# takahiroharada/OCLRadixSort

Measured on AMD Instinct MI355X. Metric: Gkeys/s on uniform-random u32 keys; achieved % of HBM-read roofline, higher is better.
Workload: dtype u32; 1 GPU; Key-only RadixSort32, 67108864 uniform-random u32 keys (splitmix64 hi32, seed 123+step), 1xMI355X, in place; keys_per_gpu=67108864, parallelism=1 GPU, sort_algo=auto, digit_bits=8

## Files before the change

oclradixsort_amd/csrc/finish16_kernels.hpp:

```cpp
#pragma once
#include <hip/hip_runtime.h>
#include <stdint.h>

#include "hybrid_kernels.hpp"

namespace adlhip {

template <int R2>
struct Finish16Cfg {
    static constexpr int CAP = 128 * R2;
    static constexpr size_t PER_WAVE = 2 * CAP + 256 * 4;
};

__device__ __forceinline__ uint32_t finish16_index(uint32_t p) { return (p & ~127u) | ((p & 63u) << 1) | ((p >> 6) & 1u); }

__device__ __forceinline__ void finish16_lds_order() { __builtin_amdgcn_fence(__ATOMIC_ACQ_REL, "wavefront"); }

template <int RR>
__device__ __forceinline__ void finish16_rows(const uint32_t* __restrict__ src32, uint32_t* __restrict__ out, uint32_t m, int lane,
                                              uint16_t* __restrict__ buf16, uint32_t* __restrict__ cnt, uint32_t low_bits, uint32_t hi)
{
    constexpr int L = RR - 1;
    const bool a_lo = 2u * (uint32_t)(64 * L + lane) < m, a_hi = 2u * (uint32_t)(64 * L + lane) + 1u < m;
    const bool b_lo = (uint32_t)(128 * L + lane) < m, b_hi = (uint32_t)(128 * L + 64 + lane) < m;
    uint32_t kp[RR];
#pragma unroll
    for (int j = 0; j < RR; ++j)
        if (j < L || a_lo) kp[j] = __builtin_nontemporal_load(src32 + j * 64 + lane);
    bool placed = false;
    const int npass = ((int)low_bits + 7) / 8;
    int sb = 0;
    const uint32_t* buf32 = reinterpret_cast<const uint32_t*>(buf16);
    for (int p = 0; p < npass; ++p) {
        const int nb = ((int)low_bits - sb + (npass - p - 1)) / (npass - p);
        const uint32_t mask = (1u << nb) - 1u;
        const bool v_lo = placed ? b_lo : a_lo, v_hi = placed ? b_hi : a_hi;
        auto dlo = [&](uint32_t x) -> uint32_t { return (x >> sb) & mask; };
        auto dhi = [&](uint32_t x) -> uint32_t { return (x >> (16 + sb)) & mask; };
        {
            const uint32_t d0 = (uint32_t)__builtin_amdgcn_readfirstlane((int)dlo(kp[0]));
            bool same = true;
#pragma unroll
            for (int j = 0; j < RR; ++j) {
                if (j < L || v_lo) same &= dlo(kp[j]) == d0;
                if (j < L || v_hi) same &= dhi(kp[j]) == d0;
            }
            if (__all(same)) {
                sb += nb;
                continue;
            }
        }
        const u32x4 z = {0u, 0u, 0u, 0u};
        *reinterpret_cast<u32x4*>(cnt + 4 * lane) = z;
        uint32_t rk[RR];
#pragma unroll
        for (int j = 0; j < RR; ++j) {
            uint32_t r0 = 0u, r1 = 0u;
            if (j < L || v_lo) r0 = __hip_atomic_fetch_add(&cnt[dlo(kp[j])], 1u, __ATOMIC_RELAXED, __HIP_MEMORY_SCOPE_WAVEFRONT);
            if (j < L || v_hi) r1 = __hip_atomic_fetch_add(&cnt[dhi(kp[j])], 1u, __ATOMIC_RELAXED, __HIP_MEMORY_SCOPE_WAVEFRONT);
            rk[j] = r0 | (r1 << 16);
        }
        {
            const u32x4 c = *reinterpret_cast<const u32x4*>(cnt + 4 * lane);
            const uint32_t s4 = c.x + c.y + c.z + c.w;
            const uint32_t ex = wave_incl_scan_u32(s4) - s4;
            u32x4 o;
            o.x = ex;
            o.y = ex + c.x;
            o.z = o.y + c.y;
            o.w = o.z + c.z;
            *reinterpret_cast<u32x4*>(cnt + 4 * lane) = o;
        }
        finish16_lds_order();
#pragma unroll
        for (int j = 0; j < RR; ++j) {
            uint32_t p0 = 0u, p1 = 0u;
            if (j < L || v_lo) p0 = cnt[dlo(kp[j])] + (rk[j] & 0xffffu);
            if (j < L || v_hi) p1 = cnt[dhi(kp[j])] + (rk[j] >> 16);
            if (j < L || v_lo) buf16[finish16_index(p0)] = (uint16_t)kp[j];
            if (j < L || v_hi) buf16[finish16_index(p1)] = (uint16_t)(kp[j] >> 16);
        }
        finish16_lds_order();
#pragma unroll
        for (int j = 0; j < RR; ++j)
            if (j < L || b_lo) kp[j] = buf32[j * 64 + lane];
        placed = true;
        sb += nb;
    }
    if (placed) {
#pragma unroll
        for (int j = 0; j < RR; ++j) {
            if (j < L || b_lo) __builtin_nontemporal_store(hi | (kp[j] & 0xffffu), out + 128 * j + lane);
            if (j < L || b_hi) __builtin_nontemporal_store(hi | (kp[j] >> 16), out + 128 * j + 64 + lane);
        }
    } else {
#pragma unroll
        for (int j = 0; j < RR; ++j) {
            if (j < L || a_lo) out[2 * (64 * j + lane)] = hi | (kp[j] & 0xffffu);
            if (j < L || a_hi) out[2 * (64 * j + lane) + 1] = hi | (kp[j] >> 16);
        }
    }
}

template <int RR, int R2>
__device__ __forceinline__ void finish16_dispatch(int rows2, const uint32_t* __restrict__ src32, uint32_t* __restrict__ out, uint32_t m,
                                                  int lane, uint16_t* __restrict__ buf16, uint32_t* __restrict__ cnt, uint32_t low_bits,
                                                  uint32_t hi)
{
    if constexpr (RR >= R2) {
        finish16_rows<R2>(src32, out, m, lane, buf16, cnt, low_bits, hi);
    } else {
        if (rows2 <= RR) finish16_rows<RR>(src32, out, m, lane, buf16, cnt, low_bits, hi);
        else finish16_dispatch<RR + 1, R2>(rows2, src32, out, m, lane, buf16, cnt, low_bits, hi);
    }
}

template <int R2, int WAVES>
__global__ __launch_bounds__(64 * WAVES) void wave_finish16_kernel(const uint16_t* __restrict__ slab, uint32_t* __restrict__ out,
                                                                    const uint32_t* __restrict__ seg_off,
                                                                    const uint32_t* __restrict__ seg_cnt, uint32_t stride,
                                                                    const uint32_t* __restrict__ gate, const uint32_t* __restrict__ dyn,
                                                                    uint32_t num_segments, uint32_t* fault)
{
    if (gate && *gate != 0u) return;
    using C = Finish16Cfg<R2>;
    extern __shared__ __attribute__((aligned(16))) unsigned char smem[];
    const int lane = (int)threadIdx.x & 63;
    const int w = (int)threadIdx.x >> 6;
    unsigned char* mine = smem + (size_t)w * C::PER_WAVE;
    uint16_t* __restrict__ buf16 = reinterpret_cast<uint16_t*>(mine);
    uint32_t* __restrict__ cnt = reinterpret_cast<uint32_t*>(mine + 2 * C::CAP);
    const uint32_t seg = (uint32_t)__builtin_amdgcn_readfirstlane((int)(blockIdx.x * (uint32_t)WAVES + (uint32_t)w));
    if (seg >= num_segments) return;
    const uint32_t low_bits = (uint32_t)__builtin_amdgcn_readfirstlane((int)dyn[0]);
    const uint32_t m = (uint32_t)__builtin_amdgcn_readfirstlane((int)seg_cnt[seg]);
    const uint32_t begin = (uint32_t)__builtin_amdgcn_readfirstlane((int)seg_off[seg]);
    if (m == 0u) return;
    if (m > (uint32_t)C::CAP || low_bits > 16u) {
        if (lane == 0) atomicOr(fault + 1, 0x40000u);
        return;
    }
    const uint32_t hi = ((dyn[1] << 16) | seg) << low_bits;
    const uint32_t* src32 = reinterpret_cast<const uint32_t*>(slab + (size_t)seg * stride);
    finish16_dispatch<1, R2>((int)((m + 127u) >> 7), src32, out + begin, m, lane, buf16, cnt, low_bits, hi);
}

}
```

Before: 215.3 Gkeys/s.

## Add single-pass 512-bin finish16 with odd-even transposition cleanup of low bits

When more than 8 low bits remain, the wave-level finisher now counting-sorts the segment on the top 9 bits in one pass instead of two 8-bit passes. Any leftover lower bits are fixed by a bounded number of odd-even transposition rounds in registers, using DPP to exchange across lanes, and it falls back to the multi-pass path when a bin is too large. The LDS tile is padded to avoid bank conflicts and the counter array is enlarged. This removes one full histogram/scan/scatter pass per segment, at the cost of more LDS per wave and the extra sort rounds.

```diff
diff --git a/oclradixsort_amd/csrc/finish16_kernels.hpp b/oclradixsort_amd/csrc/finish16_kernels.hpp
--- a/oclradixsort_amd/csrc/finish16_kernels.hpp
+++ b/oclradixsort_amd/csrc/finish16_kernels.hpp
@@ -6,15 +6,163 @@
 
 namespace adlhip {
 
+constexpr int kFinish16BinBits = 9;
+constexpr int kFinish16MaxRounds = 24;
+
 template <int R2>
 struct Finish16Cfg {
     static constexpr int CAP = 128 * R2;
-    static constexpr size_t PER_WAVE = 2 * CAP + 256 * 4;
+    static constexpr int BINS = 1 << kFinish16BinBits;
+    static constexpr size_t TILE = 256 * (R2 | 1);
+    static constexpr size_t PER_WAVE = TILE + 4 * BINS;
 };
 
 __device__ __forceinline__ uint32_t finish16_index(uint32_t p) { return (p & ~127u) | ((p & 63u) << 1) | ((p >> 6) & 1u); }
 
 __device__ __forceinline__ void finish16_lds_order() { __builtin_amdgcn_fence(__ATOMIC_ACQ_REL, "wavefront"); }
+
+template <int RR>
+__device__ __forceinline__ uint32_t finish16_block_byte(uint32_t p)
+{
+    constexpr uint32_t J = 2 * RR;
+    if constexpr ((RR & 1) != 0) {
+        return 2u * p;
+    } else if constexpr ((J & (J - 1)) == 0) {
+        return 2u * p + 4u * (p / J);
+    } else {
+        constexpr uint32_t MAGIC = (65536u + J - 1u) / J;
+        static_assert(64u * J * (MAGIC * J - 65536u) < 65536u, "the reciprocal is not exact over the tile");
+        return 2u * p + 4u * (__umul24(p, MAGIC) >> 16);
+    }
+}
+
+__device__ __forceinline__ uint32_t finish16_wave_max(uint32_t v)
+{
+    v = max(v, dpp_mov0<0x111, 0xf, 0xf>(v));
+    v = max(v, dpp_mov0<0x112, 0xf, 0xf>(v));
+    v = max(v, dpp_mov0<0x114, 0xf, 0xf>(v));
+    v = max(v, dpp_mov0<0x118, 0xf, 0xf>(v));
+    v = max(v, dpp_mov0<0x142, 0xa, 0xf>(v));
+    v = max(v, dpp_mov0<0x143, 0xc, 0xf>(v));
+    return (uint32_t)__builtin_amdgcn_readlane((int)v, 63);
+}
+
+template <int RR>
+__device__ __forceinline__ bool finish16_bins(const uint32_t (&kp)[RR], uint32_t* __restrict__ out, uint32_t m, int lane,
+                                              uint16_t* __restrict__ buf16, uint32_t* __restrict__ cnt, uint32_t low_bits, uint32_t hi,
+                                              bool a_lo, bool a_hi, bool b_lo, bool b_hi)
+{
+    constexpr int L = RR - 1, J = 2 * RR, S = RR | 1;
+    constexpr int NB = 1 << kFinish16BinBits, PL = NB / 64;
+    static_assert(PL % 4 == 0, "a lane scans its counters as u32x4");
+    const uint32_t bb = low_bits < (uint32_t)kFinish16BinBits ? low_bits : (uint32_t)kFinish16BinBits;
+    const uint32_t sh = low_bits - bb;
+    auto dlo = [&](uint32_t x) -> uint32_t { return (x >> sh) & (uint32_t)(NB - 1); };
+    auto dhi = [&](uint32_t x) -> uint32_t { return (x >> (16u + sh)) & (uint32_t)(NB - 1); };
+    {
+        const uint32_t d0 = (uint32_t)__builtin_amdgcn_readfirstlane((int)dlo(kp[0]));
+        bool same = true;
+#pragma unroll
+        for (int j = 0; j < RR; ++j) {
+            if (j < L || a_lo) same &= dlo(kp[j]) == d0;
+            if (j < L || a_hi) same &= dhi(kp[j]) == d0;
+        }
+        if (__all(same)) return false;
+    }
+    const u32x4 z = {0u, 0u, 0u, 0u};
+#pragma unroll
+    for (int q = 0; q < PL / 4; ++q) *reinterpret_cast<u32x4*>(cnt + PL * lane + 4 * q) = z;
+    uint32_t rk[RR];
+#pragma unroll
+    for (int j = 0; j < RR; ++j) {
+        uint32_t r0 = 0u, r1 = 0u;
+        if (j < L || a_lo) r0 = __hip_atomic_fetch_add(&cnt[dlo(kp[j])], 1u, __ATOMIC_RELAXED, __HIP_MEMORY_SCOPE_WAVEFRONT);
+        if (j < L || a_hi) r1 = __hip_atomic_fetch_add(&cnt[dhi(kp[j])], 1u, __ATOMIC_RELAXED, __HIP_MEMORY_SCOPE_WAVEFRONT);
+        rk[j] = r0 | (r1 << 16);
+    }
+    const bool tail = low_bits > bb;
+    uint32_t rounds;
+    {
+        u32x4 c[PL / 4];
+        uint32_t sum = 0u, big = 0u;
+#pragma unroll
+        for (int q = 0; q < PL / 4; ++q) {
+            c[q] = *reinterpret_cast<const u32x4*>(cnt + PL * lane + 4 * q);
+            sum += c[q].x + c[q].y + c[q].z + c[q].w;
+            big = max(max(big, max(c[q].x, c[q].y)), max(c[q].z, c[q].w));
+        }
+        rounds = finish16_wave_max(big);
+        if (tail && rounds > (uint32_t)kFinish16MaxRounds) return false;
+        uint32_t run = wave_incl_scan_u32(sum) - sum;
+#pragma unroll
+        for (int q = 0; q < PL / 4; ++q) {
+            u32x4 o;
+            o.x = run;
+            o.y = o.x + c[q].x;
+            o.z = o.y + c[q].y;
+            o.w = o.z + c[q].z;
+            run = o.w + c[q].w;
+            *reinterpret_cast<u32x4*>(cnt + PL * lane + 4 * q) = o;
+        }
+    }
+    unsigned char* tile = reinterpret_cast<unsigned char*>(buf16);
+    const bool sort = tail && rounds > 1u;
+    if (sort) {
+        const uint32_t p0 = m + (uint32_t)lane, p1 = p0 + 64u;
+        if (p0 < (uint32_t)(64 * J)) *reinterpret_cast<uint16_t*>(tile + finish16_block_byte<RR>(p0)) = (uint16_t)0xffffu;
+        if (p1 < (uint32_t)(64 * J)) *reinterpret_cast<uint16_t*>(tile + finish16_block_byte<RR>(p1)) = (uint16_t)0xffffu;
+    }
+    finish16_lds_order();
+#pragma unroll
+    for (int j = 0; j < RR; ++j) {
+        uint32_t p0 = 0u, p1 = 0u;
+        if (j < L || a_lo) p0 = cnt[dlo(kp[j])] + (rk[j] & 0xffffu);
+        if (j < L || a_hi) p1 = cnt[dhi(kp[j])] + (rk[j] >> 16);
+        if (j < L || a_lo) *reinterpret_cast<uint16_t*>(tile + finish16_block_byte<RR>(p0)) = (uint16_t)kp[j];
+        if (j < L || a_hi) *reinterpret_cast<uint16_t*>(tile + finish16_block_byte<RR>(p1)) = (uint16_t)(kp[j] >> 16);
+    }
+    finish16_lds_order();
+    if (sort) {
+        uint32_t* own = reinterpret_cast<uint32_t*>(tile) + S * lane;
+        uint32_t k[J];
+#pragma unroll
+        for (int j = 0; j < RR; ++j) {
+            const uint32_t w = own[j];
+            k[2 * j] = w & 0xffffu;
+            k[2 * j + 1] = w >> 16;
+        }
+        for (uint32_t r = 0u; r < rounds; r += 2u) {
+#pragma unroll
+            for (int j = 0; j < RR; ++j) {
+                const uint32_t a = k[2 * j], b = k[2 * j + 1];
+                k[2 * j] = min(a, b);
+                k[2 * j + 1] = max(a, b);
+            }
+            const uint32_t up = (uint32_t)__builtin_amdgcn_update_dpp((int)0xffffffffu, (int)k[0], 0x130, 0xf, 0xf, false);
+            const uint32_t dn = (uint32_t)__builtin_amdgcn_update_dpp(0, (int)k[J - 1], 0x138, 0xf, 0xf, false);
+#pragma unroll
+            for (int j = 0; j < RR - 1; ++j) {
+                const uint32_t a = k[2 * j + 1], b = k[2 * j + 2];
+                k[2 * j + 1] = min(a, b);
+                k[2 * j + 2] = max(a, b);
+            }
+            k[J - 1] = min(k[J - 1], up);
+            k[0] = max(k[0], dn);
+        }
+#pragma unroll
+        for (int j = 0; j < RR; ++j) own[j] = k[2 * j] | (k[2 * j + 1] << 16);
+        finish16_lds_order();
+    }
+#pragma unroll
+    for (int i = 0; i < J; ++i) {
+        if (i < 2 * L || (i == 2 * L ? b_lo : b_hi)) {
+            const uint32_t p = (uint32_t)(64 * i + lane);
+            const uint32_t v = *reinterpret_cast<const uint16_t*>(tile + finish16_block_byte<RR>(p));
+            __builtin_nontemporal_store(hi | v, out + p);
+        }
+    }
+    return true;
+}
 
 template <int RR>
 __device__ __forceinline__ void finish16_rows(const uint32_t* __restrict__ src32, uint32_t* __restrict__ out, uint32_t m, int lane,
@@ -27,6 +175,7 @@
 #pragma unroll
     for (int j = 0; j < RR; ++j)
         if (j < L || a_lo) kp[j] = __builtin_nontemporal_load(src32 + j * 64 + lane);
+    if (low_bits > 8u && finish16_bins<RR>(kp, out, m, lane, buf16, cnt, low_bits, hi, a_lo, a_hi, b_lo, b_hi)) return;
     bool placed = false;
     const int npass = ((int)low_bits + 7) / 8;
     int sb = 0;
@@ -129,7 +278,7 @@
     const int w = (int)threadIdx.x >> 6;
     unsigned char* mine = smem + (size_t)w * C::PER_WAVE;
     uint16_t* __restrict__ buf16 = reinterpret_cast<uint16_t*>(mine);
-    uint32_t* __restrict__ cnt = reinterpret_cast<uint32_t*>(mine + 2 * C::CAP);
+    uint32_t* __restrict__ cnt = reinterpret_cast<uint32_t*>(mine + C::TILE);
     const uint32_t seg = (uint32_t)__builtin_amdgcn_readfirstlane((int)(blockIdx.x * (uint32_t)WAVES + (uint32_t)w));
     if (seg >= num_segments) return;
     const uint32_t low_bits = (uint32_t)__builtin_amdgcn_readfirstlane((int)dyn[0]);
```

New measurement: 230.6 Gkeys/s, median of 6. 1.07x the previous value.
